# zhen6618/EPRecon

Measured on AMD Instinct MI355X. Metric: fragments_per_sec, higher is better.
Workload: dtype f32

## Files before the change

eprecon_amd/_lib.py:

```python
import ctypes
import os

import torch

_HERE = os.path.dirname(os.path.abspath(__file__))
LIB_PATH = os.environ.get("EPRECON_LIB_PATH") or os.path.join(_HERE, "libeprecon_hip.so")

_c = ctypes
_vp, _i, _i64, _f, _sz = _c.c_void_p, _c.c_int, _c.c_int64, _c.c_float, _c.c_size_t

SIGNATURES = {
    "eprecon_abi_version": (_i, []),
    "eprecon_build_arch": (_c.c_char_p, []),
    "eprecon_back_project_workspace_bytes": (_sz, [_i64, _i, _i, _i, _i, _i, _i]),
    "eprecon_back_project_async": (_i, [_vp, _i64, _vp, _i, _f, _vp, _i, _vp, _i, _i, _i, _i, _i, _i,
                                        _vp, _vp, _vp, _vp, _vp, _vp, _vp, _vp, _sz, _vp]),
    "eprecon_back_project": (_i, [_vp, _i64, _vp, _i, _f, _vp, _i, _vp, _i, _i, _i, _i, _i, _i, _i,
                                  _vp, _vp, _vp, _vp, _vp, _vp, _vp, _vp, _vp, _sz, _vp]),
    "eprecon_back_project_phase_async": (_i, [_i, _vp, _i64, _vp, _i, _f, _vp, _i, _vp, _i, _i, _i, _i, _i, _i,
                                              _vp, _vp, _vp, _vp, _vp, _vp, _vp, _vp, _sz, _vp]),
    "eprecon_back_project_rank_out": (_i, [_vp]),
    "eprecon_init_glue": (_i, []),
    "eprecon_profile_gather_kernel": (_c.c_char_p, []),
    "eprecon_hash_capacity": (_c.c_uint32, [_i64]),
    "eprecon_hash_table_bytes": (_sz, [_c.c_uint32]),
    "eprecon_hash_build_async": (_i, [_vp, _i64, _i, _vp, _c.c_uint32, _vp]),
    "eprecon_hash_build_dn_async": (_i, [_vp, _i64, _vp, _i, _vp, _c.c_uint32, _vp]),
    "eprecon_hash_query_async": (_i, [_vp, _c.c_uint32, _vp, _i64, _i, _vp, _vp]),
    "eprecon_hash_status": (_i, [_vp, _vp]),
    "eprecon_unique_workspace_bytes": (_sz, [_i64]),
    "eprecon_unique_coords_async": (_i, [_vp, _i64, _i, _vp, _c.c_uint32, _vp, _vp, _vp, _vp, _sz, _vp]),
    "eprecon_unique_coords_dn_async": (_i, [_vp, _i64, _vp, _i, _vp, _c.c_uint32, _vp, _vp, _vp, _vp, _sz, _vp]),
    "eprecon_unique_hierarchy_dn_async": (_i, [_vp, _i64, _vp, _i, _vp, _vp, _vp, _vp, _vp, _vp, _sz, _vp]),
    "eprecon_point_quantize_dn_async": (_i, [_vp, _i64, _vp, _f, _vp, _vp, _vp]),
    "eprecon_spvcnn_points_dn_async": (_i, [_vp, _i64, _vp, _i, _i, _vp, _i, _f, _vp, _f, _vp, _vp, _vp, _vp, _vp, _vp]),
    "eprecon_gru_stage_capacity": (_i64, [_vp, _i64, _i]),
    "eprecon_gru_stage_workspace_bytes": (_sz, [_i64]),
    "eprecon_gru_stage_begin_async": (_i, [_vp, _vp]),
    "eprecon_gru_stage_commit_async": (_i, [_vp, _vp, _vp, _vp]),
    "eprecon_kernel_map_async": (_i, [_vp, _c.c_uint32, _vp, _i64, _i, _i, _vp, _vp]),
    "eprecon_kernel_map_self_async": (_i, [_vp, _c.c_uint32, _vp, _i64, _i, _vp, _vp]),
    "eprecon_transpose_map_async": (_i, [_vp, _i64, _vp, _i, _vp, _vp]),
    "eprecon_sparse_conv_async": (_i, [_vp, _i64, _i, _vp, _i, _i64, _vp, _i, _i, _vp, _vp, _i, _i, _i, _vp]),
    "eprecon_conv_bn_partial_bytes": (_sz, [_i64, _i]),
    "eprecon_sparse_conv_fused_async": (_i, [_vp, _i64, _i, _vp, _i, _i64, _vp, _i, _i, _vp, _vp, _i, _vp, _i, _i, _i,
                                             _vp, _vp]),
    "eprecon_conv_desc_async": (_i, [_vp, _vp]),
    "eprecon_exclusive_scan_async": (_i, [_vp, _i64, _vp, _vp, _vp, _vp]),
    "eprecon_conv_desc_partial_rows": (_i64, [_vp]),
    "eprecon_bn_acc_words": (_sz, [_i]),
    "eprecon_conv_desc_takes_bn_acc": (_i, [_vp]),
    "eprecon_batchnorm_acc_affine_async": (_i, [_vp, _i, _i, _i, _f, _vp, _vp, _vp]),
    "eprecon_affine_rows_acc_async": (_i, [_vp, _i64, _i, _i, _vp, _i, _i, _f, _i, _vp, _i, _vp]),
    "eprecon_affine_rows_res_async": (_i, [_vp, _i64, _i, _i, _vp, _vp, _vp, _i, _i, _vp, _i, _vp]),
    "eprecon_batchnorm_finalize_affine_async": (_i, [_vp, _i64, _i64, _i, _vp, _vp, _f, _vp, _vp, _vp]),
    "eprecon_affine_rows_async": (_i, [_vp, _i64, _i, _i, _vp, _vp, _i, _vp, _i, _vp]),
    "eprecon_affine_pool2_rows_async": (_i, [_vp, _i, _i, _i, _i, _i, _vp, _vp, _i, _vp, _i, _vp]),
    "eprecon_affine_up2_rows_async": (_i, [_vp, _i, _i, _i, _i, _i, _vp, _vp, _i, _vp, _i, _vp]),
    "eprecon_pixel_map_async": (_i, [_i, _i, _i, _i, _vp, _vp]),
    "eprecon_batchnorm_apply_workspace_bytes": (_sz, [_i]),
    "eprecon_batchnorm_apply_partials_async": (_i, [_vp, _i64, _i, _i, _vp, _i64, _i64, _vp, _vp, _f, _vp, _i, _i, _vp, _i,
                                                    _vp, _vp, _vp, _sz, _vp]),
    "eprecon_batchnorm_apply_partials_res_async": (_i, [_vp, _i64, _i, _i, _vp, _i64, _i64, _vp, _vp, _f, _vp, _i, _vp, _vp, _i,
                                                        _vp, _i, _vp, _sz, _vp]),
    "eprecon_batchnorm_workspace_bytes": (_sz, [_i64, _i]),
    "eprecon_batchnorm_train_async": (_i, [_vp, _i64, _i, _i, _vp, _vp, _f, _vp, _i, _i, _vp, _i, _vp, _vp,
                                           _vp, _sz, _vp]),
    "eprecon_rowwise_layernorm_async": (_i, [_vp, _i64, _i, _i, _vp, _i, _vp, _vp, _f, _i, _i, _vp, _i, _vp]),
    "eprecon_init_select_workspace_bytes": (_sz, [_i, _i]),
    "eprecon_init_select_async": (_i, [_vp, _vp, _i64, _f, _i, _i, _i, _vp, _vp, _vp, _sz, _vp]),
    "eprecon_init_select_dense_async": (_i, [_vp, _vp, _i64, _vp, _i, _i, _i, _i, _f, _i, _i, _vp, _vp, _vp, _sz, _vp]),
    "eprecon_upsample_async": (_i, [_vp, _i, _vp, _i64, _i, _i, _vp, _vp, _vp]),
    "eprecon_aligned_coords_async": (_i, [_vp, _i64, _vp, _i, _f, _vp, _vp, _vp]),
# ... 114 lines not shown

_lib = None


def load():
    global _lib
    if _lib is not None:
        return _lib
    if not os.path.exists(LIB_PATH):
        raise EpreconError(
            f"{LIB_PATH} not found: build it with `python -m eprecon_amd.build` "
            "(hipcc --offload-arch=gfx950). eprecon_amd has no CPU fallback.")
    lib = ctypes.CDLL(LIB_PATH)
    for name, (res, args) in SIGNATURES.items():
        fn = getattr(lib, name)
        fn.restype = res
        fn.argtypes = args
    if lib.eprecon_abi_version() != ABI_VERSION:
        raise EpreconError("libeprecon_hip.so ABI version mismatch; rebuild")
    _lib = lib
    return lib


def check(rc, what):
    if rc == EPRECON_OK:
        return True
    if rc == EPRECON_EMPTY:
        return False
    if rc <= -1000:
        raise EpreconError(f"{what}: HIP error {-(rc + 1000)}")
    raise EpreconError(f"{what}: error {rc} "
                       "(-1 bad argument, -2 workspace too small, -3 unsupported size)")


def ptr(t):
    return None if t is None else t.data_ptr()


_raw_stream = getattr(torch._C, "_cuda_getCurrentRawStream", None)
_raw_device = getattr(torch._C, "_cuda_getDevice", None)


def current_stream():
    if _raw_stream is not None and _raw_device is not None:
        return _raw_stream(_raw_device()) or None
    return torch.cuda.current_stream().cuda_stream or None


class ViewsDesc(ctypes.Structure):
    _fields_ = [("src", (ctypes.c_void_p * 16) * 3), ("dst", ctypes.c_void_p * 3), ("channels", ctypes.c_int32 * 3),
                ("hw", ctypes.c_int32 * 3), ("levels", ctypes.c_int32), ("n_views", ctypes.c_int32)]


class GtCropDesc(ctypes.Structure):
    _fields_ = ([(n, ctypes.c_void_p * 3) for n in ("tsdf_full", "rgb_full", "semantic_full", "instance_full")]
                + [("full_dims", (ctypes.c_int32 * 3) * 3), ("levels", ctypes.c_int32), ("dims", ctypes.c_int32 * 3),
                   ("voxel_size", ctypes.c_float), ("origin_partial", ctypes.c_float * 3), ("old_origin", ctypes.c_float * 3),
                   ("transform", ctypes.c_float * 12)]
                + [(n, ctypes.c_void_p * 3) for n in ("tsdf_out", "rgb_out", "semantic_out", "instance_out")])


class ConvDesc(ctypes.Structure):
    _fields_ = [("x", ctypes.c_void_p), ("n_in", ctypes.c_int64), ("ld_x", ctypes.c_int),
                ("nbr", ctypes.c_void_p), ("kvol", ctypes.c_int), ("n_out", ctypes.c_int64),
                ("weight", ctypes.c_void_p), ("cin", ctypes.c_int), ("cout", ctypes.c_int),
                ("bias", ctypes.c_void_p),
                ("residual", ctypes.c_void_p), ("ld_res", ctypes.c_int),
                ("out", ctypes.c_void_p), ("ld_out", ctypes.c_int),
                ("relu", ctypes.c_int), ("accumulate", ctypes.c_int),
                ("in_scale", ctypes.c_void_p), ("in_shift", ctypes.c_void_p), ("in_relu", ctypes.c_int),
                ("res_scale", ctypes.c_void_p), ("res_shift", ctypes.c_void_p), ("res_relu", ctypes.c_int),
                ("bn_partial", ctypes.c_void_p), ("bn_ld", ctypes.c_int),
                ("ln", ctypes.c_int), ("ln_gamma", ctypes.c_void_p), ("ln_beta", ctypes.c_void_p),
                ("ln_eps", ctypes.c_float), ("ln_post_relu", ctypes.c_int),
                ("img_h", ctypes.c_int), ("img_w", ctypes.c_int), ("img_maps", ctypes.c_int),
                ("vox_rank", ctypes.c_void_p), ("grid_x", ctypes.c_int), ("grid_y", ctypes.c_int), ("grid_z", ctypes.c_int),
                ("packed_weight", ctypes.c_void_p), ("packed_weight16", ctypes.c_void_p),
                ("workspace", ctypes.c_void_p), ("workspace_bytes", ctypes.c_size_t),
                ("bn_acc", ctypes.c_void_p), ("bn_acc_ld", ctypes.c_int), ("bn_acc_c0", ctypes.c_int),
                ("bn_gamma", ctypes.c_void_p), ("bn_beta", ctypes.c_void_p),
                ("in_acc", ctypes.c_void_p), ("in_acc_ld", ctypes.c_int), ("in_acc_c0", ctypes.c_int),
                ("in_eps", ctypes.c_float), ("in_affine_scratch", ctypes.c_void_p)]


class GruStageDesc(ctypes.Structure):
    _fields_ = [("map", ctypes.c_void_p), ("target_map", ctypes.c_void_p),
                ("cur_coords", ctypes.c_void_p), ("cur_feat", ctypes.c_void_p), ("n_cur", ctypes.c_int64), ("ld_cur", ctypes.c_int),
                ("dim", ctypes.c_int), ("interval", ctypes.c_int), ("activity_mode", ctypes.c_int),
                ("rel", ctypes.c_int32 * 3),
                ("tsdf_gt", ctypes.c_void_p), ("occ_gt", ctypes.c_void_p),
                ("origin", ctypes.c_void_p), ("w2ac", ctypes.c_void_p),
                ("voxel_size", ctypes.c_float), ("resolution", ctypes.c_float),
                ("ch_voxel", ctypes.c_int), ("batch_index", ctypes.c_int),
                ("capacity", ctypes.c_int64),
                ("updated", ctypes.c_void_p), ("out_coords", ctypes.c_void_p), ("r_coords", ctypes.c_void_p),
                ("hx_voxel", ctypes.c_void_p), ("hx_image", ctypes.c_void_p), ("tsdf_target", ctypes.c_void_p),
                ("scaled1", ctypes.c_void_p), ("vox1", ctypes.c_void_p), ("inverse1", ctypes.c_void_p), ("uniq1", ctypes.c_void_p),
                ("table1", ctypes.c_void_p),
                ("scaled2", ctypes.c_void_p), ("vox2", ctypes.c_void_p), ("inverse2", ctypes.c_void_p), ("uniq2", ctypes.c_void_p),
                ("table2", ctypes.c_void_p),
                ("table_capacity", ctypes.c_uint32),
                ("counts", ctypes.c_void_p),
                ("workspace", ctypes.c_void_p), ("workspace_bytes", ctypes.c_size_t)]


class DecoderLayerDesc(ctypes.Structure):
# ... 178 lines not shown
```

eprecon_amd/back_project.py:

```python
import ctypes

import torch
import torch.nn as nn

from . import _lib

MODE_MEAN, MODE_MEAN_DEPTH, MODE_VARIANCE = 0, 1, 2
LAYOUT_NCHW, LAYOUT_NHWC = 0, 1


def mark_dense(coords, dims, interval, batch=1):
    coords._eprecon_dense = (tuple(int(d) for d in dims), int(interval), int(batch))
    return coords


def dense_rank_buffer(coords, dims, interval):
    tag = getattr(coords, "_eprecon_dense", None)
    want = (tuple(int(d) for d in dims), int(interval), 1)
    if tag != want or not coords.is_cuda or coords.shape[0] != want[0][0] * want[0][1] * want[0][2]:
        return None
    if not _lib.load().eprecon_init_glue():
        return None
    return torch.empty(coords.shape[0] + 1, dtype=torch.int32, device=coords.device)

# ... 48 lines not shown
    res = {"feats": cut(t["feats"]), "coords": cut(t["coords"]), "count": t["count"], "n_valid": n_valid,
           "n_valid_per_batch": per_batch}
    if want_grid:
        res["grid"] = cut(t["grid"], v * 2).view(v, n_valid, 2)
        res["mask"] = cut(t["mask"], v).view(v, n_valid).bool()
    if want_mean:
        res["mean"] = cut(t["mean"])
    return res


class PendingBackProject:

    def __init__(self, tensors, n, v, c, batch, min_valid_per_batch, read, want_grid, want_mean):
        self._t, self._n, self._v, self._c, self._batch = tensors, n, v, c, batch
        self._min_valid, self._read = min_valid_per_batch, read
        self._want_grid, self._want_mean = want_grid, want_mean

    def result(self):
        return self.result_from(self._read.result())

    def result_from(self, counts):
        if any(x < self._min_valid for x in counts[1:]):
            return None
        return _result(self._t, self._v, counts[0], counts[1:], self._want_grid, self._want_mean)


class CountedBackProject:

    def __init__(self, shape, inputs, count, n_valid_dev, ws, stream):
        self.shape, self.inputs, self.count, self.n_valid_dev, self.ws, self.stream = shape, inputs, count, n_valid_dev, ws, stream


def count_async(coords, origin, voxel_size, feats_shape, krcam, min_view, mode=MODE_MEAN, stream=None):
    lib = _lib.load()
    dev = coords.device
    shape = v, b, c, h, w = tuple(int(x) for x in feats_shape)
    inputs = _prep_inputs(coords, origin, krcam, v, b, dev)
    n = coords.shape[0]
    count = torch.empty((n,), dtype=torch.float32, device=dev)
    n_valid_dev = torch.empty((1 + b,), dtype=torch.int32, device=dev)
    ws = torch.empty((lib.eprecon_back_project_workspace_bytes(n, b, v, c, h, w, LAYOUT_NHWC),), dtype=torch.uint8, device=dev)

    def queue():
        _lib.check(lib.eprecon_back_project_phase_async(
            1, *_lib_args(inputs, voxel_size, None, LAYOUT_NHWC, shape, min_view, mode, {"count": count}, n_valid_dev, ws)),
            "eprecon_back_project_phase_async")
    if stream is None:
        queue()
    else:
        stream.wait_stream(torch.cuda.current_stream(dev))
        with torch.cuda.stream(stream):
            queue()
    return CountedBackProject(shape, inputs + (float(voxel_size), int(min_view), mode), count, n_valid_dev, ws, stream)


def run_async(coords, origin, voxel_size, feats, krcam, min_view, mode=MODE_MEAN, min_valid_per_batch=1,
              want_grid=False, want_mean=False, hold_read=False, extra_words=0, rank_out=None, counted=None):
    lib = _lib.load()
    dev = feats.device
    shape = v, b, c, h, w = tuple(feats.shape)
    inputs = _prep_inputs(coords, origin, krcam, v, b, dev)
    n = coords.shape[0]
    feats_c, layout = _prep_feats(feats)
    t = _alloc_outputs(n, v, c, mode, want_grid, want_mean, dev, count=None if counted is None else counted.count)
    if counted is not None:
        assert layout == LAYOUT_NHWC and counted.shape == shape and not extra_words
        assert counted.inputs[3:] == (float(voxel_size), int(min_view), mode) and counted.count.shape[0] == n
        inputs, n_valid_dev, ws = counted.inputs[:3], counted.n_valid_dev, counted.ws
        if counted.stream is not None:
            torch.cuda.current_stream(dev).wait_stream(counted.stream)
    else:
        n_valid_dev = torch.empty((1 + b + int(extra_words),), dtype=torch.int32, device=dev)
        ws = _lib.workspace(lib.eprecon_back_project_workspace_bytes(n, b, v, c, h, w, layout), dev)
    _arm_rank(lib, rank_out, n, b)
    args = _lib_args(inputs, voxel_size, feats_c, layout, shape, min_view, mode, t, n_valid_dev, ws)
    if counted is not None:
        _lib.check(lib.eprecon_back_project_phase_async(2, *args), "eprecon_back_project_phase_async")
    else:
        _lib.check(lib.eprecon_back_project_async(*args), "eprecon_back_project_async")
    read = None if hold_read else _lib.PinnedRead(n_valid_dev[:1 + b])
    t["_keep"] = (*inputs, feats_c, n_valid_dev, ws if counted is not None else None)
    pend = PendingBackProject(t, n, v, c, b, int(min_valid_per_batch), read, want_grid, want_mean)
    pend.n_valid_dev, pend.coords_all = n_valid_dev, t["coords"]
    return pend


def run(coords, origin, voxel_size, feats, krcam, min_view, mode=MODE_MEAN, min_valid_per_batch=1,
        want_grid=False, want_mean=False, rank_out=None):
    lib = _lib.load()
    dev = feats.device
    shape = v, b, c, h, w = tuple(feats.shape)
    inputs = _prep_inputs(coords, origin, krcam, v, b, dev)
    n = coords.shape[0]
    feats_c, layout = _prep_feats(feats)
    t = _alloc_outputs(n, v, c, mode, want_grid, want_mean, dev)
    n_valid_dev = torch.empty((1 + b,), dtype=torch.int32, device=dev)
    ws = _lib.workspace(lib.eprecon_back_project_workspace_bytes(n, b, v, c, h, w, layout), dev)

    if min_view <= 0 and b == 1 and n >= max(int(min_valid_per_batch), 1):
        _arm_rank(lib, rank_out, n, b)
        _lib.check(lib.eprecon_back_project_async(
            *_lib_args(inputs, voxel_size, feats_c, layout, shape, min_view, mode, t, n_valid_dev, ws)), "eprecon_back_project_async")
        _lib.defer_check(n_valid_dev[0:1], n, "back-projection with min_view <= 0: rows with a batch index out of range")
        return _result(t, v, n, [n], want_grid, want_mean, sliced=False)
    n_valid_host = (ctypes.c_int32 * (1 + b))()
    _lib.count_host_read()
# ... 79 lines not shown
```

eprecon_amd/csrc/back_project.hip:

```cpp
#include <stdlib.h>

#include "back_project_common.hpp"

namespace {
using namespace ep;


struct BpParams {
    const int32_t *coords;
    int n;
    const float *origin;
    int batch;
    float voxel_size;
    const float *feats_nhwc;
    const float *krcam;
    int V, C, H, W;
    int Cs;
    int min_view;
    float *out_feats;
    float *out_mean;
    int32_t *out_coords;
    float *count;
    float *out_grid;
    uint8_t *out_mask;
// ... 526 lines not shown
        for (int s = kWave / 2; s > 0; s >>= 1) x += __shfl_xor(x, s);
        __syncthreads();
        if (lane == 0) sRed[wid] = x;
        __syncthreads();
        float t = 0.f;
#pragma unroll
        for (int w = 0; w < 1024 / kWave; ++w) t += sRed[w];
        return t;
    };
    float s = 0.f, m = 0.f;
    for (int j = tid; j < len; j += 1024) {
        const float x = d[(size_t)j * cout];
        if (x > 0.f) { s += x; m += 1.f; }
    }
    const float tot = block_sum(s), cntp = block_sum(m);
    const float mu = tot / cntp;
    float ss = 0.f;
    for (int j = tid; j < len; j += 1024) {
        const float x = d[(size_t)j * cout];
        if (x > 0.f) ss = fmaf(x - mu, x - mu, ss);
    }
    const float sigma = sqrtf(block_sum(ss)) + 1e-5f;
    for (int j = tid; j < len; j += 1024) {
        const float x = d[(size_t)j * cout];
        d[(size_t)j * cout] = x > 0.f ? (x - mu) / sigma : 0.f;
    }
}

template <bool VEC4>
__global__ __launch_bounds__(256) void nchw_to_nhwc_kernel(const float *__restrict__ in,
                                                           float *__restrict__ out, int C, int hw, int Cs,
                                                           int32_t *zero = nullptr, int zero_n = 0)
{
    extern __shared__ __attribute__((aligned(16))) char smem[];
    if (blockIdx.x == 0 && blockIdx.y == 0 && (int)threadIdx.x < zero_n) zero[threadIdx.x] = 0;
    relayout_body<VEC4>(smem, in, out, C, hw, Cs, (int)blockIdx.y, (int)blockIdx.x * kTrPix);
}

template <int VOX, bool VEC4>
__global__ __launch_bounds__(256) void bp_prepare_kernel(BpParams p, int32_t *tile_sums, int32_t *blk_batch,
                                                         const float *__restrict__ in, float *__restrict__ out, int hw,
                                                         int tiles, int R)
{
    extern __shared__ __attribute__((aligned(16))) char smem[];
    const int bid = blockIdx.x;
    if (bid < R) {
        const int map = bid / tiles;
        relayout_body<VEC4>(smem, in, out, p.C, hw, p.Cs, map, (bid - map * tiles) * kTrPix);
    } else {
        count_body<VOX>(smem, p, tile_sums, blk_batch, bid - R);
    }
}

size_t gather_lds_bytes(bool mlp, int vox, int V, int B)
{
    const size_t nP = ((size_t)V * B * 12 + 3) & ~(size_t)3;
    return (size_t)vox * V * (mlp ? 12 : 8) + nP * 4 + (size_t)vox * (mlp ? 3 : 5) * 4 + (size_t)(256 / kWave) * 4 * 3;
}

template <int VOX, int MODE>
int launch_gather(const BpParams &p, bool mlp, hipStream_t st)
{
    const size_t lds = gather_lds_bytes(mlp, VOX, p.V, p.batch);
    const dim3 grid(p.ntile), block(256);
    if (p.C % 4 != 0) {
        hipLaunchKernelGGL((bp_gather_kernel<VOX, MODE, 1, 0>), grid, block, lds, st, p);
    } else {
        pick<6, 8, 10, 20, 0>(p.C / 4, [&](auto qt) {
            constexpr int QT = decltype(qt)::value;
            if (mlp) hipLaunchKernelGGL((bp_gather_mlp_kernel<VOX, MODE, QT, 1>), grid, block, lds, st, p);
            else hipLaunchKernelGGL((bp_gather_kernel<VOX, MODE, 4, QT>), grid, block, lds, st, p);
            return 0;
        });
    }
    EP_LAUNCH_CHECK();
    return EPRECON_OK;
}

thread_local int32_t *t_rank_out = nullptr;

struct BpArgs {
    int phase; const int32_t *coords; int64_t n; const float *origin; int batch; float voxel_size;
    const float *feats; int feats_layout; const float *krcam; int n_views, channels, height, width, min_view, mode;
    float *out_feats, *out_mean; int32_t *out_coords; float *count, *out_grid; uint8_t *out_mask; int32_t *n_valid_dev;
    void *workspace; size_t workspace_bytes; void *stream;
    int32_t *rank;
};

int bp_validate(BpArgs &a)
{
    a.rank = nullptr;
    if (a.phase != EPRECON_BP_COUNT) {
        a.rank = t_rank_out;
        t_rank_out = nullptr;
    }
    if (a.rank && a.batch != 1) return EPRECON_ERR_ARG;
    if (a.phase != 0 && a.feats_layout != EPRECON_LAYOUT_NHWC) return EPRECON_ERR_ARG;
    if (a.phase == EPRECON_BP_COUNT && !a.feats) a.feats = a.krcam;
    if (a.n < 0 || a.n > 0x7fffffff / 64 || a.batch <= 0 || a.n_views <= 0 || a.n_views > 32 || a.channels <= 0 ||
        a.height <= 1 || a.width <= 1 || a.mode < 0 || a.mode > 2)
        return EPRECON_ERR_ARG;
    if (!a.origin || !a.feats || !a.krcam || !a.n_valid_dev || !a.workspace) return EPRECON_ERR_ARG;
    if (a.n > 0 && (!a.coords || !a.count || (a.phase != EPRECON_BP_COUNT && (!a.out_feats || !a.out_coords))))
        return EPRECON_ERR_ARG;
    if ((size_t)a.n_views * a.batch * 12 * sizeof(float) > 32 * 1024) return EPRECON_ERR_UNSUPPORTED;
    if (a.workspace_bytes < eprecon_back_project_workspace_bytes(a.n, a.batch, a.n_views, a.channels, a.height, a.width,
// ... 87 lines not shown
        }
        hipLaunchKernelGGL((bp_count_kernel<VOX>), dim3(pl.nblk_count), dim3(256), pl.lds_count, st, p, pl.tile_sums, pl.blk_batch);
    }
    EP_LAUNCH_CHECK();
    if (!p.fold) {
        hipLaunchKernelGGL(bp_scan_kernel, dim3(1), dim3(1024), 0, st, pl.tile_sums, pl.ntile, a.n_valid_dev,
                           (const int32_t *)pl.blk_batch, pl.nblk_count, a.batch);
        EP_LAUNCH_CHECK();
    }
    return EPRECON_OK;
}

template <int VOX>
int bp_queue_gather(const BpArgs &a, const BpPlan &pl)
{
    hipStream_t st = (hipStream_t)a.stream;
    if (a.n == 0) {
        if (a.rank) EP_HIP_CHECK(hipMemsetAsync(a.rank, 0, sizeof(int32_t), st));
        return EPRECON_OK;
    }
    int rc = ep::profile_bracket_begin(st);
    if (rc != EPRECON_OK) return rc;
    rc = pick<EPRECON_BP_MEAN, EPRECON_BP_MEAN_DEPTH, EPRECON_BP_VARIANCE>(
        a.mode, [&](auto mode) { return launch_gather<VOX, decltype(mode)::value>(pl.p, pl.mlp, st); });
    if (rc != EPRECON_OK) return rc;
    rc = ep::profile_bracket_end(st, pl.mlp ? "bp_gather_mlp_kernel" : "bp_gather_kernel");
    if (rc != EPRECON_OK) return rc;
    if (a.mode == EPRECON_BP_MEAN_DEPTH) {
        hipLaunchKernelGGL(bp_depth_norm_kernel, dim3(a.batch), dim3(1024), 0, st, a.out_feats, a.channels + 1, a.n_valid_dev);
        EP_LAUNCH_CHECK();
    }
    return EPRECON_OK;
}

template <int VOX>
int bp_queue(const BpArgs &a, const BpPlan &pl)
{
    const int rc = a.phase != EPRECON_BP_GATHER ? bp_queue_count<VOX>(a, pl) : EPRECON_OK;
    return rc != EPRECON_OK || a.phase == EPRECON_BP_COUNT ? rc : bp_queue_gather<VOX>(a, pl);
}

int bp_async_impl(BpArgs a)
{
    const int rc = bp_validate(a);
    if (rc != EPRECON_OK) return rc;
    const BpPlan pl = bp_plan(a);
    switch (pl.vox) {
        case 256: return bp_queue<256>(a, pl);
        case 64: return bp_queue<64>(a, pl);
        default: return bp_queue<16>(a, pl);
    }
}

}

extern "C" {

size_t eprecon_back_project_workspace_bytes(int64_t n, int batch, int n_views, int channels,
                                            int height, int width, int feats_layout)
{
    size_t bytes = ep::align_up((size_t)ep::ceil_div(n > 0 ? n : 1, 16) * sizeof(int32_t), 256);
    bytes += ep::align_up((size_t)ep::ceil_div(n > 0 ? n : 1, 256) * (batch > 0 ? batch : 1) * sizeof(int32_t), 256);
    if (feats_layout == EPRECON_LAYOUT_NCHW)
        bytes += ep::align_up((size_t)n_views * batch * channels * height * width * sizeof(float), 256);
    return bytes + 256;
}

int eprecon_nchw_to_nhwc_async(const float *in, float *out, int maps, int channels, int hw,
                               void *stream)
{
    if (!in || !out || maps <= 0 || channels <= 0 || hw <= 0) return EPRECON_ERR_ARG;
    const size_t lds = (size_t)channels * (kTrPix + 1) * sizeof(float);
    if (lds > 64 * 1024) return EPRECON_ERR_UNSUPPORTED;
    const dim3 grid((unsigned)ep::ceil_div(hw, kTrPix), (unsigned)maps);
    if (relayout_vec4(in, out, hw, channels))
        hipLaunchKernelGGL(nchw_to_nhwc_kernel<true>, grid, dim3(256), lds, (hipStream_t)stream, in, out, channels, hw, channels,
                           (int32_t *)nullptr, 0);
    else
        hipLaunchKernelGGL(nchw_to_nhwc_kernel<false>, grid, dim3(256), lds, (hipStream_t)stream, in, out, channels, hw, channels,
                           (int32_t *)nullptr, 0);
    EP_LAUNCH_CHECK();
    return EPRECON_OK;
}

int eprecon_back_project_rank_out(int32_t *rank) { t_rank_out = rank; return EPRECON_OK; }

int eprecon_init_glue(void) { return ep::switch_off("EPRECON_INIT_GLUE") ? 0 : 1; }

int eprecon_back_project_async(const int32_t *coords, int64_t n, const float *origin, int batch, float voxel_size, const float *feats,
                               int feats_layout, const float *krcam, int n_views, int channels, int height, int width,
                               int min_view, int mode, float *out_feats, float *out_mean, int32_t *out_coords, float *count,
                               float *out_grid, uint8_t *out_mask, int32_t *n_valid_dev, void *workspace, size_t workspace_bytes,
                               void *stream)
{
    return bp_async_impl({0, coords, n, origin, batch, voxel_size, feats, feats_layout, krcam, n_views, channels, height, width,
                          min_view, mode, out_feats, out_mean, out_coords, count, out_grid, out_mask, n_valid_dev, workspace,
                          workspace_bytes, stream, nullptr});
}

int eprecon_back_project_phase_async(int phase, const int32_t *coords, int64_t n, const float *origin, int batch, float voxel_size,
                                     const float *feats, int feats_layout, const float *krcam, int n_views, int channels,
                                     int height, int width, int min_view, int mode, float *out_feats, float *out_mean,
                                     int32_t *out_coords, float *count, float *out_grid, uint8_t *out_mask, int32_t *n_valid_dev,
                                     void *workspace, size_t workspace_bytes, void *stream)
{
    if (phase != EPRECON_BP_COUNT && phase != EPRECON_BP_GATHER) return EPRECON_ERR_ARG;
    return bp_async_impl({phase, coords, n, origin, batch, voxel_size, feats, feats_layout, krcam, n_views, channels, height, width,
                          min_view, mode, out_feats, out_mean, out_coords, count, out_grid, out_mask, n_valid_dev, workspace,
                          workspace_bytes, stream, nullptr});
}

int eprecon_back_project(const int32_t *coords, int64_t n, const float *origin, int batch, float voxel_size, const float *feats,
                         int feats_layout, const float *krcam, int n_views, int channels, int height, int width, int min_view,
                         int mode, int min_valid_per_batch, float *out_feats, float *out_mean, int32_t *out_coords, float *count,
                         float *out_grid, uint8_t *out_mask, int32_t *n_valid_dev, int32_t *n_valid_host, void *workspace,
                         size_t workspace_bytes, void *stream)
{
    if (!n_valid_host) return EPRECON_ERR_ARG;
    const int rc = eprecon_back_project_async(coords, n, origin, batch, voxel_size, feats, feats_layout, krcam, n_views, channels,
                                              height, width, min_view, mode, out_feats, out_mean, out_coords, count, out_grid,
                                              out_mask, n_valid_dev, workspace, workspace_bytes, stream);
    if (rc != EPRECON_OK) return rc;
    hipStream_t st = (hipStream_t)stream;
    EP_HIP_CHECK(hipMemcpyAsync(n_valid_host, n_valid_dev, sizeof(int32_t) * (size_t)(1 + batch), hipMemcpyDeviceToHost, st));
    EP_HIP_CHECK(hipStreamSynchronize(st));
    for (int b = 0; b < batch; ++b)
        if (n_valid_host[1 + b] < min_valid_per_batch) return EPRECON_EMPTY;
    return EPRECON_OK;
}

}
```

eprecon_amd/fragment_step.py:

```python
import os

import torch

from . import _lib
from . import back_project as BP
from . import grid_ops as GO
from . import synthetic as S
from .config import CH_IMG, CH_INIT_DOWN, N_VIEWS
from .occupancy_initialization import Occupancy_Initialization

LEVELS = [("bp24", 2, 4, 2), ("bp48", 1, 2, 0), ("bp96", 0, 1, 0)]


class Cfg2Step:
    def __init__(self, seed=0, device=None, height=480, width=640, n_vox=(96, 96, 96)):
        self.device = device or torch.device("cuda")
        self.seed = seed
        self.window = S.make_window(seed=seed, width=width, height=height, n_vox=n_vox)
        self.shapes = S.pyramid_shapes(height, width)
        dev = self.device
        t = lambda a: torch.from_numpy(a).to(dev)
        self.origin = t(self.window["vol_origin_partial"][None].copy())
        self.voxel_size = self.window["voxel_size"]
        self.krcam = [t(self.window["proj_matrices"][:, l][:, None].copy()) for l in range(3)]
        self.feats = [t(S.make_features(1000 * seed + 10 + l, N_VIEWS, self.shapes[l])) for l in range(3)]
        f1 = [t(S.make_features(1000 * seed + 20 + l, N_VIEWS, self.shapes[l])) for l in range(3)]
        self.features_init = [[f1[l][v] for l in range(3)] for v in range(N_VIEWS)]
        self.coords = {iv: BP.mark_dense(t(S.dense_coords(n_vox, iv)), [n // iv for n in n_vox], iv) for iv in (4, 2, 1)}
        self.shape_init = tuple(n // 2 for n in n_vox)
        torch.manual_seed(1234)
        self.init_net = Occupancy_Initialization(CH_IMG, CH_INIT_DOWN, N_VIEWS).to(dev)
        self.init_net.train()
        self.last = {}
        self.defer_reads = False
        self._inflight = None
        self.levels_inside = True
        self.profile_dominant = False
        self.bp_side_stream = False
        self._bp_stream = None

    @torch.no_grad()
    def run(self):
        issued = self._issue()
        if not self.defer_reads:
            return self._finish(issued)
        prev, self._inflight = self._inflight, issued
        return self._finish(prev) if prev is not None else {}

    def flush(self):
        if self._inflight is not None:
            prev, self._inflight = self._inflight, None
            return self._finish(prev)
        return self.last

    def _finish(self, issued):
        out, pending, select = issued
        if select is not None:
            out["stage0_coords"], _ = select.result()
        for name in pending:
            out[name] = pending[name].result()
        self.last = out
        return out

    def _issue(self):
        out = {}
        pending = {}
        main = torch.cuda.current_stream(self.device)
        side = self._bp_stream if self.bp_side_stream else main

        def queue_levels():
            if side is not main:
                side.wait_stream(main)
            with torch.cuda.stream(side):
                for name, lvl, interval, mv in LEVELS:
                    if self.profile_dominant and name == "bp96":
                        _lib.load().eprecon_profile_enable(2)
                    pending[name] = BP.run_async(self.coords[interval], self.origin, self.voxel_size, self.feats[lvl],
                                                 self.krcam[lvl], mv)

        if not self.levels_inside:
            queue_levels()
        init = self.init_net(self.coords[2], self.origin, self.voxel_size, self.features_init,
                             self.krcam[1], self.shape_init, 1, 2, between=queue_levels if self.levels_inside else None)
        out["init"] = init
        select = None
        if init is not None:
            select = GO.init_select_async(init[0], init[1], 1, dim=self.shape_init[0] // 2, cell=4, dense=self.init_net.dense_map)
        if side is not main:
            main.wait_stream(side)
        return out, pending, select

    def dominant_kernel_ms(self, lib):
        return float(lib.eprecon_profile_gather_ms())

    def dominant_kernel_bytes(self):
        c, h, w = self.shapes[0]
        n = self.coords[1].shape[0]
        nv = self.last["bp96"]["n_valid"] if self.last.get("bp96") else n
        return 16 * n + 4 * N_VIEWS * c * h * w + nv * (4 * c + 16)

    def dominant_kernel_l1_bandwidth(self, launch_ms):
        if not launch_ms:
            return None
        c = self.shapes[0][0]
        n = self.coords[1].shape[0]
        nv = self.last["bp96"]["n_valid"] if self.last.get("bp96") else n
        req = float(nv) * N_VIEWS * 4 * 4 * c
        peak = 64.0 * 256 * 2.4e9 / 1e12
        ach = req / (launch_ms * 1e-3) / 1e12
        return {"requested_bytes": req, "requested_note": "upper bound: every valid voxel visible in all views (4 taps x 4 C bytes per view)",
                "achieved_TBps": ach, "peak_TBps": peak, "frac": ach / peak}

    def describe(self):
        return {"workload": "cfg2: one 9-view 640x480 window, 96^3 FBV: Occupancy_Initialization on the dense "
                            "48^3 grid (2D fusion convs + variance volume + submanifold stack) + stage-0 "
                            "selection + Back_Project on dense 24^3/48^3/96^3 (C=80/40/24)",
                "views": N_VIEWS, "image": "640x480", "n_vox": list(self.window["n_vox"]),
                "stages": ["occupancy_init48", "init_select"] + [l[0] for l in LEVELS],
                "weights": "seeded random", "fragments_per_step_per_gpu": 1,
                "host_reads": ("counts of step k read after step k + 1 is queued (flushed inside the timed region)"
                               if self.defer_reads else "every step reads its own counts before returning")}


# ... 269 lines not shown
```

include/eprecon_hip.h:

```cpp
#ifndef EPRECON_HIP_H
#define EPRECON_HIP_H

#include <stddef.h>
#include <stdint.h>

#ifdef __cplusplus
extern "C" {
#endif

#define EPRECON_OK 0
#define EPRECON_EMPTY 1
#define EPRECON_ERR_ARG (-1)
#define EPRECON_ERR_WORKSPACE (-2)
#define EPRECON_ERR_UNSUPPORTED (-3)
#define EPRECON_ERR_HIP_BASE (-1000)

#define EPRECON_ABI_VERSION 1
int eprecon_abi_version(void);
const char *eprecon_build_arch(void);

#define EPRECON_BP_MEAN 0
#define EPRECON_BP_MEAN_DEPTH 1
#define EPRECON_BP_VARIANCE 2

#define EPRECON_LAYOUT_NCHW 0
#define EPRECON_LAYOUT_NHWC 1

size_t eprecon_back_project_workspace_bytes(int64_t n, int batch, int n_views, int channels,
                                            int height, int width, int feats_layout);

int eprecon_back_project_async(const int32_t *coords, int64_t n, const float *origin, int batch,
                               float voxel_size, const float *feats, int feats_layout,
                               const float *krcam, int n_views, int channels, int height,
                               int width, int min_view, int mode, float *out_feats,
                               float *out_mean, int32_t *out_coords, float *count,
                               float *out_grid, uint8_t *out_mask, int32_t *n_valid_dev,
                               void *workspace, size_t workspace_bytes, void *stream);

int eprecon_back_project(const int32_t *coords, int64_t n, const float *origin, int batch,
                         float voxel_size, const float *feats, int feats_layout,
                         const float *krcam, int n_views, int channels, int height, int width,
                         int min_view, int mode, int min_valid_per_batch, float *out_feats,
                         float *out_mean, int32_t *out_coords, float *count, float *out_grid,
                         uint8_t *out_mask, int32_t *n_valid_dev, int32_t *n_valid_host,
                         void *workspace, size_t workspace_bytes, void *stream);

#define EPRECON_BP_COUNT 1
#define EPRECON_BP_GATHER 2
int eprecon_back_project_phase_async(int phase, const int32_t *coords, int64_t n, const float *origin, int batch,
                                     float voxel_size, const float *feats, int feats_layout,
                                     const float *krcam, int n_views, int channels, int height,
                                     int width, int min_view, int mode, float *out_feats,
                                     float *out_mean, int32_t *out_coords, float *count,
                                     float *out_grid, uint8_t *out_mask, int32_t *n_valid_dev,
                                     void *workspace, size_t workspace_bytes, void *stream);

int eprecon_back_project_rank_out(int32_t *rank);

int eprecon_init_glue(void);

int eprecon_profile_enable(int on);
float eprecon_profile_gather_ms(void);
const char *eprecon_profile_gather_kernel(void);

int eprecon_profile_conv_arm(int kvol, int cin, int cout, int64_t min_rows);
float eprecon_profile_conv_ms(int64_t *rows_out, const char **kernel_out);
int64_t eprecon_profile_conv_pairs(void);
int64_t eprecon_profile_conv_executed_pairs(void);
const char *eprecon_profile_last_conv_kernel(void);
int eprecon_profile_mark_async(int id, void *stream);

int eprecon_nchw_to_nhwc_async(const float *in, float *out, int maps, int channels, int hw,
                               void *stream);
typedef struct eprecon_views_desc {
    const float *src[3][16];
    float *dst[3];
    int32_t channels[3]; int32_t hw[3];
    int32_t levels; int32_t n_views;
} eprecon_views_desc;
int eprecon_views_to_rows_async(const eprecon_views_desc *desc, void *stream);

uint32_t eprecon_hash_capacity(int64_t n);
size_t eprecon_hash_table_bytes(uint32_t capacity);
int eprecon_hash_build_async(const int32_t *coords, int64_t n, int quantum, void *table,
                             uint32_t capacity, void *stream);
int eprecon_hash_build_dn_async(const int32_t *coords, int64_t n_cap, const int32_t *n_dev, int quantum, void *table,
                                uint32_t capacity, void *stream);
int eprecon_hash_query_async(const void *table, uint32_t capacity, const int32_t *queries, int64_t m,
                             int quantum, int32_t *out_index, void *stream);
int eprecon_hash_status(const void *table, void *stream);

size_t eprecon_unique_workspace_bytes(int64_t n);
int eprecon_exclusive_scan_async(const int32_t *in, int64_t n, int32_t *out, int32_t *total, int32_t *scratch, void *stream);
int eprecon_unique_coords_async(const int32_t *coords, int64_t n, int quantum, void *table,
                                uint32_t capacity, int32_t *inverse, int32_t *unique_coords,
                                int32_t *n_unique_dev, void *workspace, size_t workspace_bytes,
                                void *stream);

int eprecon_unique_coords_dn_async(const int32_t *coords, int64_t n_cap, const int32_t *n_dev, int quantum, void *table,
                                   uint32_t capacity, int32_t *inverse, int32_t *unique_coords, int32_t *n_unique_dev,
                                   void *workspace, size_t workspace_bytes, void *stream);
int eprecon_unique_hierarchy_dn_async(const int32_t *coords, int64_t n_cap, const int32_t *n_dev, int levels, void *const *tables,
                                      const uint32_t *capacities, int32_t *const *inverse, int32_t *const *unique_coords,
                                      int32_t *summary, void *workspace, size_t workspace_bytes, void *stream);

int eprecon_kernel_map_self_async(const void *table, uint32_t capacity, const int32_t *coords, int64_t n, int stride, int32_t *nbr,
                                  void *stream);
int eprecon_kernel_map_async(const void *table, uint32_t capacity, const int32_t *coords, int64_t n,
// ... 430 lines not shown
```

Before: 798.8.

## Batch back-projection relayout and count phases for all levels into one launch

Adds a multi-level prepare entry point that runs the NCHW-to-NHWC relayout and the voxel count phase for up to four back-projection levels in a single grid, with each block picking its level from a table. It also batches the per-level valid-count readbacks into one shared buffer and a single pinned host read. The aim is to cut kernel launch overhead and the multiple host syncs across levels. It adds block-dispatch branching and a max-LDS launch, and only runs when levels_inside is set and the side stream is off.

```diff
diff --git a/eprecon_amd/_lib.py b/eprecon_amd/_lib.py
--- a/eprecon_amd/_lib.py
+++ b/eprecon_amd/_lib.py
@@ -19,6 +19,9 @@
                                   _vp, _vp, _vp, _vp, _vp, _vp, _vp, _vp, _vp, _sz, _vp]),
     "eprecon_back_project_phase_async": (_i, [_i, _vp, _i64, _vp, _i, _f, _vp, _i, _vp, _i, _i, _i, _i, _i, _i,
                                               _vp, _vp, _vp, _vp, _vp, _vp, _vp, _vp, _sz, _vp]),
+    "eprecon_back_project_prepare_levels_async": (_i, [_vp, _i, _vp]),
+    "eprecon_back_project_workspace_maps_offset": (_sz, [_i64, _i]),
+    "eprecon_bp_levels": (_i, []),
     "eprecon_back_project_rank_out": (_i, [_vp]),
     "eprecon_init_glue": (_i, []),
     "eprecon_profile_gather_kernel": (_c.c_char_p, []),
@@ -239,6 +242,14 @@
                 ("hw", ctypes.c_int32 * 3), ("levels", ctypes.c_int32), ("n_views", ctypes.c_int32)]
 
 
+class BpLevel(ctypes.Structure):
+    _fields_ = [("coords", ctypes.c_void_p), ("n", ctypes.c_int64), ("origin", ctypes.c_void_p), ("batch", ctypes.c_int32),
+                ("voxel_size", ctypes.c_float), ("feats", ctypes.c_void_p), ("feats_layout", ctypes.c_int32),
+                ("krcam", ctypes.c_void_p), ("n_views", ctypes.c_int32), ("channels", ctypes.c_int32), ("height", ctypes.c_int32),
+                ("width", ctypes.c_int32), ("min_view", ctypes.c_int32), ("mode", ctypes.c_int32), ("count", ctypes.c_void_p),
+                ("n_valid_dev", ctypes.c_void_p), ("workspace", ctypes.c_void_p), ("workspace_bytes", ctypes.c_size_t)]
+
+
 class GtCropDesc(ctypes.Structure):
     _fields_ = ([(n, ctypes.c_void_p * 3) for n in ("tsdf_full", "rgb_full", "semantic_full", "instance_full")]
                 + [("full_dims", (ctypes.c_int32 * 3) * 3), ("levels", ctypes.c_int32), ("dims", ctypes.c_int32 * 3),
diff --git a/eprecon_amd/back_project.py b/eprecon_amd/back_project.py
--- a/eprecon_amd/back_project.py
+++ b/eprecon_amd/back_project.py
@@ -124,6 +124,77 @@
         with torch.cuda.stream(stream):
             queue()
     return CountedBackProject(shape, inputs + (float(voxel_size), int(min_view), mode), count, n_valid_dev, ws, stream)
+
+
+class PreparedMaps:
+
+    def __init__(self, nhwc, ws, stream):
+        self.nhwc, self.ws, self.stream = nhwc, ws, stream
+
+
+class PendingLevels:
+
+    def __init__(self, pends, handles):
+        self._pends, self._offsets, self._host = list(pends), [hd.n_valid_off for hd in handles], None
+        assert len(self._pends) == len(self._offsets) and all(hd.n_valid_all is handles[0].n_valid_all for hd in handles)
+        assert all(p.n_valid_dev.data_ptr() == hd.n_valid_dev.data_ptr() for p, hd in zip(self._pends, handles))
+        self._read = _lib.PinnedRead(handles[0].n_valid_all)
+
+    def results(self):
+        if self._host is None:
+            self._host = self._read.result()
+        return [p.result_from(self._host[o:o + 1 + p._batch]) for p, o in zip(self._pends, self._offsets)]
+
+
+def prepare_levels_async(levels, stream=None):
+    lib = _lib.load()
+    if not 1 <= len(levels) <= 4:
+        raise _lib.EpreconError("prepare_levels_async takes one to four levels")
+    dev = levels[0][3].device
+    rows = []
+    for lv in levels:
+        coords, origin, voxel_size, feats, krcam, min_view = lv[:6]
+        mode = lv[6] if len(lv) > 6 else MODE_MEAN
+        shape = tuple(int(x) for x in feats.shape)
+        feats_c, layout = _prep_feats(feats)
+        inputs = None if coords is None else _prep_inputs(coords, origin, krcam, shape[0], shape[1], dev)
+        rows.append((shape, feats_c, layout, inputs, float(voxel_size), int(min_view), mode))
+    n_valid_all = torch.empty((sum(1 + r[0][1] for r in rows if r[3] is not None),), dtype=torch.int32, device=dev)
+    descs = (_lib.BpLevel * len(rows))()
+    handles, off = [], 0
+    for d, (shape, feats_c, layout, inputs, voxel_size, min_view, mode) in zip(descs, rows):
+        v, b, c, h, w = shape
+        n = 0 if inputs is None else inputs[0].shape[0]
+        ws = torch.empty((lib.eprecon_back_project_workspace_bytes(n, b, v, c, h, w, layout),), dtype=torch.uint8, device=dev)
+        d.n, d.batch, d.voxel_size, d.feats, d.feats_layout = n, b, voxel_size, feats_c.data_ptr(), layout
+        d.n_views, d.channels, d.height, d.width, d.min_view, d.mode = v, c, h, w, min_view, mode
+        d.workspace, d.workspace_bytes = ws.data_ptr(), ws.numel()
+        nhwc = feats_c
+        if layout == LAYOUT_NCHW:
+            o = lib.eprecon_back_project_workspace_maps_offset(n, b)
+            nhwc = ws[o:o + 4 * v * b * c * h * w].view(torch.float32).view(v, b, h, w, c).permute(0, 1, 4, 2, 3)
+        if inputs is None:
+            handles.append(PreparedMaps(nhwc, (ws, feats_c), stream))
+            continue
+        count = torch.empty((n,), dtype=torch.float32, device=dev)
+        n_valid_dev = n_valid_all[off:off + 1 + b]
+        d.coords, d.origin, d.krcam = (x.data_ptr() for x in inputs)
+        d.count, d.n_valid_dev = count.data_ptr(), n_valid_dev.data_ptr()
+        hd = CountedBackProject(shape, inputs + (voxel_size, min_view, mode), count, n_valid_dev, ws, stream)
+        hd.nhwc, hd.feats, hd.n_valid_all, hd.n_valid_off = nhwc, feats_c, n_valid_all, off
+        handles.append(hd)
+        off += 1 + b
+
+    def queue():
+        _lib.check(lib.eprecon_back_project_prepare_levels_async(ctypes.byref(descs), len(rows), _lib.current_stream()),
+                   "eprecon_back_project_prepare_levels_async")
+    if stream is None:
+        queue()
+    else:
+        stream.wait_stream(torch.cuda.current_stream(dev))
+        with torch.cuda.stream(stream):
+            queue()
+    return handles
 
 
 def run_async(coords, origin, voxel_size, feats, krcam, min_view, mode=MODE_MEAN, min_valid_per_batch=1,
diff --git a/eprecon_amd/csrc/back_project.hip b/eprecon_amd/csrc/back_project.hip
--- a/eprecon_amd/csrc/back_project.hip
+++ b/eprecon_amd/csrc/back_project.hip
@@ -602,6 +602,45 @@
     }
 }
 
+constexpr int kMaxLevels = 4;
+struct BpLevelDev {
+    int end_relayout, end;
+    int vox, vec4, hw, tiles;
+    const float *in;
+    float *out;
+    int32_t *tile_sums, *blk_batch;
+    BpParams p;
+};
+struct BpLevelTable {
+    BpLevelDev lv[kMaxLevels];
+};
+
+__global__ __launch_bounds__(256) void bp_prepare_levels_kernel(BpLevelTable t)
+{
+    extern __shared__ __attribute__((aligned(16))) char smem[];
+    const int bid = blockIdx.x;
+    int l = 0, begin = 0;
+#pragma unroll
+    for (int k = 0; k + 1 < kMaxLevels; ++k) {
+        const int e = t.lv[k].end;
+        if (bid >= e) {
+            l = k + 1;
+            begin = e;
+        }
+    }
+    const BpLevelDev &L = t.lv[l];
+    if (bid < L.end_relayout) {
+        const int r = bid - begin, map = r / L.tiles, p0 = (r - map * L.tiles) * kTrPix;
+        if (L.vec4) relayout_body<true>(smem, L.in, L.out, L.p.C, L.hw, L.p.Cs, map, p0);
+        else relayout_body<false>(smem, L.in, L.out, L.p.C, L.hw, L.p.Cs, map, p0);
+    } else {
+        const int cb = bid - L.end_relayout;
+        if (L.vox == 256) count_body<256>(smem, L.p, L.tile_sums, L.blk_batch, cb);
+        else if (L.vox == 64) count_body<64>(smem, L.p, L.tile_sums, L.blk_batch, cb);
+        else count_body<16>(smem, L.p, L.tile_sums, L.blk_batch, cb);
+    }
+}
+
 size_t gather_lds_bytes(bool mlp, int vox, int V, int B)
 {
     const size_t nP = ((size_t)V * B * 12 + 3) & ~(size_t)3;
@@ -795,6 +834,105 @@
     }
 }
 
+BpArgs level_args(const eprecon_bp_level &lv, void *stream)
+{
+    return {EPRECON_BP_COUNT, lv.coords, lv.n, lv.origin, lv.batch, lv.voxel_size, lv.feats, lv.feats_layout, lv.krcam, lv.n_views,
+            lv.channels, lv.height, lv.width, lv.min_view, lv.mode, nullptr, nullptr, nullptr, lv.count, nullptr, nullptr,
+            lv.n_valid_dev, lv.workspace, lv.workspace_bytes, stream, nullptr};
+}
+
+int bp_validate_level(BpArgs &a, bool listed)
+{
+    if (a.feats_layout != EPRECON_LAYOUT_NCHW && a.feats_layout != EPRECON_LAYOUT_NHWC) return EPRECON_ERR_ARG;
+    if (listed && a.feats_layout == EPRECON_LAYOUT_NHWC && !a.feats) a.feats = a.krcam;
+    if (a.n < 0 || a.n > 0x7fffffff / 64 || a.batch <= 0 || a.n_views <= 0 || a.n_views > 32 || a.channels <= 0 ||
+        a.height <= 1 || a.width <= 1 || a.mode < 0 || a.mode > 2)
+        return EPRECON_ERR_ARG;
+    if (!a.feats || !a.workspace) return EPRECON_ERR_ARG;
+    if (listed && (!a.origin || !a.krcam || !a.n_valid_dev || (a.n > 0 && !a.count))) return EPRECON_ERR_ARG;
+    if ((size_t)a.n_views * a.batch * 12 * sizeof(float) > 32 * 1024) return EPRECON_ERR_UNSUPPORTED;
+    if (a.workspace_bytes < eprecon_back_project_workspace_bytes(a.n, a.batch, a.n_views, a.channels, a.height, a.width,
+                                                                 a.feats_layout))
+        return EPRECON_ERR_WORKSPACE;
+    if ((size_t)a.n_views * a.batch * a.channels * a.height * a.width > 0x7fffffffull) return EPRECON_ERR_UNSUPPORTED;
+    return EPRECON_OK;
+}
+
+int bp_prepare_levels_impl(const eprecon_bp_level *levels, int n_levels, hipStream_t st)
+{
+    if (!levels || n_levels <= 0 || n_levels > kMaxLevels) return EPRECON_ERR_ARG;
+    BpArgs args[kMaxLevels];
+    BpPlan plans[kMaxLevels];
+    bool listed[kMaxLevels];
+    for (int l = 0; l < n_levels; ++l) {
+        args[l] = level_args(levels[l], st);
+        listed[l] = levels[l].coords != nullptr;
+        const int rc = bp_validate_level(args[l], listed[l]);
+        if (rc != EPRECON_OK) return rc;
+        plans[l] = bp_plan(args[l]);
+        if (plans[l].nchw && plans[l].lds_relayout > 64 * 1024) return EPRECON_ERR_UNSUPPORTED;
+    }
+    if (!eprecon_bp_levels() || plans[0].chain4) {
+        for (int l = 0; l < n_levels; ++l) {
+            const BpArgs &a = args[l];
+            const BpPlan &pl = plans[l];
+            int rc = EPRECON_OK;
+            if (listed[l]) rc = pl.vox == 256 ? bp_queue_count<256>(a, pl) : (pl.vox == 64 ? bp_queue_count<64>(a, pl) : bp_queue_count<16>(a, pl));
+            else if (pl.nchw)
+                rc = eprecon_nchw_to_nhwc_async(a.feats, pl.nhwc, a.n_views * a.batch, a.channels, a.height * a.width, st);
+            if (rc != EPRECON_OK) return rc;
+        }
+        return EPRECON_OK;
+    }
+    BpLevelTable t;
+    size_t lds = 0;
+    int cursor = 0;
+    for (int l = 0; l < kMaxLevels; ++l) {
+        BpLevelDev &d = t.lv[l];
+        d = BpLevelDev{};
+        if (l < n_levels) {
+            const BpArgs &a = args[l];
+            const BpPlan &pl = plans[l];
+            const bool count = listed[l] && a.n > 0;
+            if (listed[l] && a.n == 0)
+                EP_HIP_CHECK(hipMemsetAsync(a.n_valid_dev, 0, sizeof(int32_t) * (size_t)(1 + a.batch), st));
+            d.hw = a.height * a.width;
+            d.tiles = ep::ceil_div(d.hw, kTrPix);
+            d.vox = pl.vox;
+            d.vec4 = relayout_vec4(a.feats, pl.nhwc, d.hw, pl.p.Cs) ? 1 : 0;
+            d.in = a.feats; d.out = pl.nhwc; d.tile_sums = pl.tile_sums; d.blk_batch = pl.blk_batch;
+            d.p = pl.p;
+            const bool relayout = pl.nchw && (count || !listed[l]);
+            if (relayout) {
+                cursor += d.tiles * a.n_views * a.batch;
+                lds = pl.lds_relayout > lds ? pl.lds_relayout : lds;
+            }
+            d.end_relayout = cursor;
+            if (count) {
+                cursor += pl.nblk_count;
+                lds = pl.lds_count > lds ? pl.lds_count : lds;
+            }
+        } else {
+            d.end_relayout = cursor;
+        }
+        d.end = cursor;
+    }
+    if (cursor > 0) {
+        hipLaunchKernelGGL(bp_prepare_levels_kernel, dim3((unsigned)cursor), dim3(256), lds, st, t);
+        EP_LAUNCH_CHECK();
+    }
+    for (int l = 0; l < n_levels; ++l) {
+        const BpArgs &a = args[l];
+        const BpPlan &pl = plans[l];
+        if (listed[l] && a.n > 0 && !pl.p.fold) {
+            hipLaunchKernelGGL(bp_scan_kernel, dim3(1), dim3(1024), 0, st, pl.tile_sums, pl.ntile, a.n_valid_dev,
+                               (const int32_t *)pl.blk_batch, pl.nblk_count, a.batch);
+            EP_LAUNCH_CHECK();
+        }
+    }
+    return EPRECON_OK;
+}
+
 }
 
 extern "C" {
@@ -872,4 +1010,17 @@
     return EPRECON_OK;
 }
 
-}
+size_t eprecon_back_project_workspace_maps_offset(int64_t n, int batch)
+{
+    return ep::align_up((size_t)ep::ceil_div(n, 16) * sizeof(int32_t), 256) +
+           ep::align_up((size_t)ep::ceil_div(n, 256) * batch * sizeof(int32_t), 256);
+}
+
+int eprecon_bp_levels(void) { return ep::switch_off("EPRECON_BP_LEVELS") ? 0 : 1; }
+
+int eprecon_back_project_prepare_levels_async(const eprecon_bp_level *levels, int n_levels, void *stream)
+{
+    return bp_prepare_levels_impl(levels, n_levels, (hipStream_t)stream);
+}
+
+}
diff --git a/eprecon_amd/fragment_step.py b/eprecon_amd/fragment_step.py
--- a/eprecon_amd/fragment_step.py
+++ b/eprecon_amd/fragment_step.py
@@ -38,6 +38,7 @@
         self.profile_dominant = False
         self.bp_side_stream = False
         self._bp_stream = None
+        self.levels_beside_2d = False
 
     @torch.no_grad()
     def run(self):
@@ -58,7 +59,11 @@
         if select is not None:
             out["stage0_coords"], _ = select.result()
         for name in pending:
-            out[name] = pending[name].result()
+            if name == "_levels":
+                names, read = pending[name]
+                out.update(zip(names, read.results()))
+            else:
+                out[name] = pending[name].result()
         self.last = out
         return out
 
@@ -68,7 +73,26 @@
         main = torch.cuda.current_stream(self.device)
         side = self._bp_stream if self.bp_side_stream else main
 
+        one_launch = self.levels_inside and not self.bp_side_stream and bool(_lib.load().eprecon_bp_levels())
+
+        def prepare_levels(stream):
+            return BP.prepare_levels_async(
+                [(self.coords[interval], self.origin, self.voxel_size, self.feats[lvl], self.krcam[lvl], mv)
+                 for _, lvl, interval, mv in LEVELS], stream=stream)
+        beside = self.levels_beside_2d or os.environ.get("EPRECON_BP_LEVELS_BESIDE", "0") == "1"
+        early = prepare_levels(_lib.side_stream(self.device, _lib.SIDE_SETUP)) if one_launch and beside else None
+
         def queue_levels():
+            if one_launch:
+                handles = early if early is not None else prepare_levels(None)
+                pends = []
+                for (name, lvl, interval, mv), hd in zip(LEVELS, handles):
+                    if self.profile_dominant and name == "bp96":
+                        _lib.load().eprecon_profile_enable(2)
+                    pends.append(BP.run_async(self.coords[interval], self.origin, self.voxel_size, hd.nhwc, self.krcam[lvl], mv,
+                                              hold_read=True, counted=hd))
+                pending["_levels"] = ([l[0] for l in LEVELS], BP.PendingLevels(pends, handles))
+                return
             if side is not main:
                 side.wait_stream(main)
             with torch.cuda.stream(side):
diff --git a/include/eprecon_hip.h b/include/eprecon_hip.h
--- a/include/eprecon_hip.h
+++ b/include/eprecon_hip.h
@@ -54,6 +54,25 @@
                                      float *out_mean, int32_t *out_coords, float *count,
                                      float *out_grid, uint8_t *out_mask, int32_t *n_valid_dev,
                                      void *workspace, size_t workspace_bytes, void *stream);
+
+typedef struct eprecon_bp_level {
+    const int32_t *coords;
+    int64_t n;
+    const float *origin;
+    int32_t batch;
+    float voxel_size;
+    const float *feats;
+    int32_t feats_layout;
+    const float *krcam;
+    int32_t n_views, channels, height, width, min_view, mode;
+    float *count;
+    int32_t *n_valid_dev;
+    void *workspace;
+    size_t workspace_bytes;
+} eprecon_bp_level;
+int eprecon_back_project_prepare_levels_async(const eprecon_bp_level *levels, int n_levels, void *stream);
+size_t eprecon_back_project_workspace_maps_offset(int64_t n, int batch);
+int eprecon_bp_levels(void);
 
 int eprecon_back_project_rank_out(int32_t *rank);
 
```

Result: faster. 820.5, median of 6 (+2.7%).
